# lbcb-sci/raven

Hardware: AMD Instinct MI355X
Metric: read Gbase/s through overlap+polish (higher is better)
Workload: dtype u32

## Files before the change

raven_amd/csrc/poa4.hip:

```cpp
#include <algorithm>
#include <cstddef>
#include <cstdio>
#include <cstdlib>
#include <cstring>
#include <vector>

#include "poa.h"
#include "poa2_window.h"

namespace rvn {

namespace {

struct P4 {
  static constexpr int G = 4, GS = 16, kBand = 32;
  static constexpr int kRing = 22;
  static constexpr int kRowB = 64;
  static constexpr int kMaxD = 8;
  static constexpr int kEdges = 8;
  static constexpr int kEdgesMax = 15;
  static constexpr int kU = 8;
};
constexpr u32 kNone4 = 0xFFFFu;
constexpr i32 kNegU = -0x30000000;
// ... 187 lines not shown
#if defined(__HIP_DEVICE_COMPILE__)
  asm volatile("" : "+v"(p));
#endif
  return p;
}

__host__ __device__ inline u32 group_min_u(u32 v) {
#pragma unroll
  for (int off = 8; off > 0; off >>= 1) {
    const u32 o = static_cast<u32>(sv::bperm(static_cast<int>(v), sv::lane() ^ off));
    v = o < v ? o : v;
  }
  return v;
}
__host__ __device__ inline i32 group_max_i(i32 v) {
#pragma unroll
  for (int off = 8; off > 0; off >>= 1) {
    const i32 o = sv::bperm(v, sv::lane() ^ off);
    v = o > v ? o : v;
  }
  return v;
}

__host__ __device__ inline u32 poa4_nth_pred_rank(const Poa4Slot& sl, u32 v, u32 k, bool full) {
  const Poa2Slot& g = sl.g;
  const u32 c = g.in_cnt[v];
  u32 seen = 0;
  for (u32 i = 0; i < c; ++i) {
    const u32 t = g.in_tail[v * kPoaMaxIn + i];
    if (full || g.mark[t]) {
      if (seen == k) return sl.rb[t] & 0xFFFFu;
      ++seen;
    }
  }
  return 0;
}

__host__ __device__ __forceinline__ u32 mulhi_u32(u32 a, u32 b) {
#if defined(__HIP_DEVICE_COMPILE__)
  return __umulhi(a, b);
#else
  return static_cast<u32>((static_cast<unsigned long long>(a) * b) >> 32);
#endif
}
__host__ __device__ __forceinline__ u32 magic_of(u32 d) { return d <= 1 ? 0u : static_cast<u32>(0x100000000ULL / d) + 1u; }
__host__ __device__ __forceinline__ u32 div_magic(u32 n, u32 m) { return m ? mulhi_u32(n, m) : n; }

struct alignas(16) Poa4LdsDesc {
  u32 segtab[32];
  u32 seq2[60];
  u8 bytes[1024];
};

__host__ __device__ inline void poa4_guide_to_lds(Poa4LdsDesc& S, const PoaLayer* Lp, u32 len, i32 span) {
  const int lane = sv::lane();
  if (lane < 8) {
    const i32 sg = lane;
    const i32 x0 = (sg * span) / 8, x1 = ((sg + 1) * span) / 8;
    const i32 wa = sg == 0 ? 0 : static_cast<i32>(Lp->way[sg - 1]);
    const i32 wb = sg == 7 ? static_cast<i32>(len) : static_cast<i32>(Lp->way[sg]);
    S.segtab[4 * sg] = static_cast<u32>(x0);
    S.segtab[4 * sg + 1] = static_cast<u32>(wa);
    S.segtab[4 * sg + 2] = static_cast<u32>(wb - wa);
    S.segtab[4 * sg + 3] = magic_of(static_cast<u32>(x1 > x0 ? x1 - x0 : 1));
  }
}
template <class K>
__host__ __device__ __forceinline__ i32 poa4_band_start(const Poa4LdsDesc& S, i32 bpos, i32 lb, i32 span, u32 span_magic, u32 len) {
  i32 x = bpos - lb;
  x = x < 0 ? 0 : (x > span ? span : x);
  const u32 seg = div_magic(static_cast<u32>(x) * 8u, span_magic);
  const u32 sg = seg > 7u ? 7u : seg;
  const uint4 st = *reinterpret_cast<const uint4*>(&S.segtab[4 * sg]);
  const i32 dw = static_cast<i32>(st.z);
  const u32 num = static_cast<u32>(x - static_cast<i32>(st.x)) * static_cast<u32>(dw < 0 ? -dw : dw);
  const i32 qn = static_cast<i32>(div_magic(num, st.w));
  i32 b = static_cast<i32>(st.y) + (dw < 0 ? -qn : qn) - K::kBand / 2;
  const i32 bmax = static_cast<i32>(len) + 1 - K::kBand;
  b = b > bmax ? bmax : b;
  b = b < 0 ? 0 : b;
  return (b == bmax && bmax > 0) ? (b + 1) & ~1 : b & ~1;
}

struct Poa4ScoresAny {
  i32 m, n, g;
  __host__ __device__ explicit Poa4ScoresAny(const Poa4Args& A) : m(A.m), n(A.n_), g(A.gp) {}
};
struct Poa4ScoresRacon {
  static constexpr i32 m = 3, n = -5, g = -4;
  __host__ __device__ explicit Poa4ScoresRacon(const Poa4Args&) {}
};
template <class K, class SC>
__host__ __device__ inline void poa4_dp(const Poa4Args A, Poa4Lds& S, unsigned char* slot_mem, bool act, u32 t_end, u32 len,
                                        u32& best_rho1) {
  P4_ASSUME_GLOBAL(slot_mem);
  P4_ASSUME_LDS(&S);
  const int lane = sv::lane();
  const int gl = lane & 15, q = lane >> 4;
  const Poa4Slot sl = poa4_carve(slot_mem, A.nmax, A.lmax);
  {
    const u32 neg = pack16(kNegInf16, kNegInf16);
    for (int idx = gl; idx < K::kRing * kRowW4; idx += 16) lds_st32(S, poa4_ring_byte(q, static_cast<u32>(idx)), neg);
    if (lane < 40) S.neg[lane] = neg;
#if !defined(__HIP_DEVICE_COMPILE__) && defined(RVN_DEBUG_KNOBS)
    if (const char* f = knob("RVN_POA4_RING_FILL")) {
      const int mode = std::atoi(f);
      for (int idx = gl; idx < K::kRing * kRowW4; idx += 16) {
        u32 h = (static_cast<u32>(idx) * 2654435761u) ^ (static_cast<u32>(q) * 40503u) ^ (len * 97u);
        h ^= h >> 13;
        const i32 base = mode == 3 ? 10 : -100, span = mode == 3 ? 50 : 800;
        const i32 lo = mode == 2 ? 28000 : base - static_cast<i32>(h % span), hi = mode == 2 ? 28000 : base - static_cast<i32>((h >> 12) % span);
        if (mode >= 1 && mode <= 3) lds_st32(S, poa4_ring_byte(q, static_cast<u32>(idx)), pack16(lo, hi));
      }
// ... 503 lines not shown
    g.visits[i] = blen >= 2 ? 1 : 0;
    g.order[i] = static_cast<u16>(i);
    rb[i] = i | (i << 16);
    const i32 wgt = poa_layer_weight(A.src, bb, i);
    if (i > 0) {
      const i32 wp = poa_layer_weight(A.src, bb, i - 1);
      g.in_cnt[i] = 1;
      g.in_tail[i * kPoaMaxIn] = static_cast<u16>(i - 1);
      g.in_w[i * kPoaMaxIn] = wp + wgt;
    } else {
      g.in_cnt[i] = 0;
    }
    g.out_cnt[i] = i + 1 < blen ? 1 : 0;
  }
  for (u32 i = blen + lane; i < A.nmax; i += 64) {
    g.in_cnt[i] = 0;
    g.out_cnt[i] = 0;
    g.visits[i] = 0;
  }
  sv::sync();
  return 1;
}

template <class GT>
__host__ __device__ __forceinline__ u32 poa4_letter(const GT& Sg, u32 p) {
  return (Sg.seq2[(p + 1) >> 4] >> (2 * ((p + 1) & 15u))) & 3u;
}

__host__ __device__ __forceinline__ Poa2Slot poa4_graph(unsigned char* slot_mem, u32 nmax, u32 lmax, bool flip) {
  Poa2Slot g = poa4_carve(slot_mem, nmax, lmax).g;
  if (flip) {
    u16* t = g.order;
    g.order = g.order2;
    g.order2 = t;
  }
  return g;
}
__host__ __device__ __forceinline__ void atomic_add_i32(i32* p, i32 v) {
#if defined(__HIP_DEVICE_COMPILE__)
  __hip_atomic_fetch_add(p, v, __ATOMIC_RELAXED, __HIP_MEMORY_SCOPE_WORKGROUP);
#else
  *p += v;
#endif
}
__host__ __device__ __forceinline__ void atomic_inc_u16(u16* base, u32 idx) {
#if defined(__HIP_DEVICE_COMPILE__)
  __hip_atomic_fetch_add(reinterpret_cast<u32*>(base) + (idx >> 1), (idx & 1u) ? 0x10000u : 1u, __ATOMIC_RELAXED,
                         __HIP_MEMORY_SCOPE_WORKGROUP);
#else
  base[idx] += 1;
#endif
}

template <int GW, int UP>
__host__ __device__ inline u32 poa4_update_graph(const Poa4Args A, u16* nslot, const u32* seq2, unsigned char* slot_mem, bool act,
                                                 const PoaLayer* Lp, u32 len, u32 lb, u32& nn, bool& flip,
                                                 unsigned long long& t_add, unsigned long long& t_ord) {
  P4_ASSUME_GLOBAL(slot_mem);
  P4_ASSUME_GLOBAL(Lp);
  P4_ASSUME_LDS(nslot);
  P4_ASSUME_LDS(seq2);
  const int lane = sv::lane();
  const int gl = lane & (GW - 1), gbase = lane & ~(GW - 1);
  constexpr unsigned long long kGMask = GW == 64 ? ~0ULL : ((1ULL << (GW & 63)) - 1ULL);
  auto shift1 = [&](int v, int fill) -> int {
    if constexpr (GW == 16) {
      return sv::row_shr<1>(v, fill);
    } else {
      const int t = sv::bperm(v, lane - 1);
      return gl == 0 ? fill : t;
    }
  };
  auto gmax = [&](i32 v) -> i32 {
    if constexpr (GW == 16) return group_max_i(v);
    else return sv::wave_max(v);
  };
  const Poa2Slot g = poa4_graph(slot_mem, A.nmax, A.lmax, flip);
  const u32* const rb32 = poa4_carve(slot_mem, A.nmax, A.lmax).rb;
  u16* const rb16 = reinterpret_cast<u16*>(poa4_carve(slot_mem, A.nmax, A.lmax).rb);
  const PoaLayer L = *Lp;
  const u32 nmax = A.nmax, lmax = A.lmax;
  unsigned long long t0 = sv::clock();
  const u32 n_old = nn;
  const u32 max_len = static_cast<u32>(sv::wave_max(act ? static_cast<int>(len) : 0));
  auto gballot = [&](bool p) -> unsigned long long { return (sv::ballot(p) >> gbase) & kGMask; };
  auto letter_at = [&](u32 p) -> u32 { return (seq2[(p + 1) >> 4] >> (2 * ((p + 1) & 15u))) & 3u; };
  u32 first_p = 0xFFFFFFFFu;
  for (u32 p0 = 0; p0 < max_len; p0 += UP * GW) {
    if (!sv::any(act && first_p == 0xFFFFFFFFu && p0 < len)) break;
    u32 pn[UP];
#pragma unroll
    for (int u = 0; u < UP; ++u) {
      const u32 p = p0 + static_cast<u32>(GW) * static_cast<u32>(u) + static_cast<u32>(gl);
      pn[u] = (act && p < len) ? g.pos_node[p] : kNone4;
    }
#pragma unroll
    for (int u = 0; u < UP; ++u) {
      const unsigned long long bal = gballot(pn[u] != kNone4);
      if (first_p == 0xFFFFFFFFu && bal) first_p = p0 + static_cast<u32>(GW) * static_cast<u32>(u) + static_cast<u32>(__builtin_ctzll(bal));
    }
  }
  u32 carry_slot = n_old, carry_b = lb;
  if (act && first_p != 0xFFFFFFFFu) {
    const u32 an = g.pos_node[first_p];
    const u32 rb_an = rb32[an];
    u32 r = rb_an & 0xFFFFu;
    const u32 ac = g.al_cnt[an];
    const uint2 al2 = *reinterpret_cast<const uint2*>(g.al + static_cast<size_t>(an) * 4);
    const u32 a0 = al2.x & 0xFFFFu, a1 = al2.x >> 16, a2 = al2.y & 0xFFFFu;
    const u32 r0 = rb32[ac > 0 ? a0 : an] & 0xFFFFu, r1 = rb32[ac > 1 ? a1 : an] & 0xFFFFu, r2 = rb32[ac > 2 ? a2 : an] & 0xFFFFu;
    r = r0 < r ? r0 : r;
    r = r1 < r ? r1 : r;
    r = r2 < r ? r2 : r;
    carry_slot = r;
    carry_b = rb_an >> 16;
  }
  u32 total_new = 0;
  u32 why = 0;
  u32 prev_tgt = kNone4;
  i32 prev_w = 0;
  for (u32 p0 = 0; p0 < max_len; p0 += UP * GW) {
    const bool go = act && why == 0;
    u32 p[UP], an[UP], letter[UP];
    bool valid[UP], has[UP];
#pragma unroll
    for (int u = 0; u < UP; ++u) {
      p[u] = p0 + static_cast<u32>(GW) * static_cast<u32>(u) + static_cast<u32>(gl);
      valid[u] = go && p[u] < len;
      an[u] = valid[u] ? g.pos_node[p[u]] : kNone4;
      letter[u] = valid[u] ? letter_at(p[u]) : 0u;
    }
    u32 c_an[UP], ac[UP], rk_an[UP], bp_an[UP];
    uint2 al2[UP];
    i32 wgt[UP];
#pragma unroll
    for (int u = 0; u < UP; ++u) {
      has[u] = valid[u] && an[u] != kNone4;
      const u32 a = has[u] ? an[u] : 0u;
      c_an[u] = g.code[a];
      ac[u] = g.al_cnt[a];
      const u32 rba = rb32[a];
      rk_an[u] = rba & 0xFFFFu;
      bp_an[u] = rba >> 16;
      al2[u] = *reinterpret_cast<const uint2*>(g.al + static_cast<size_t>(a) * 4);
      wgt[u] = valid[u] ? static_cast<i32>(static_cast<u8>(poa_layer_weight(A.src, L, p[u]))) : 0;
    }
    u32 kt[UP][3], c_kt[UP][3], rk_kt[UP][3];
#pragma unroll
    for (int u = 0; u < UP; ++u) {
      if (!has[u]) ac[u] = 0;
      kt[u][0] = al2[u].x & 0xFFFFu;
      kt[u][1] = al2[u].x >> 16;
      kt[u][2] = al2[u].y & 0xFFFFu;
#pragma unroll
      for (int k = 0; k < 3; ++k) {
        const u32 t = static_cast<u32>(k) < ac[u] ? kt[u][k] : 0u;
        c_kt[u][k] = g.code[t];
        rk_kt[u][k] = rb32[t] & 0xFFFFu;
      }
    }
    u32 tgt[UP], id_new[UP];
    bool is_new[UP];
#pragma unroll
    for (int u = 0; u < UP; ++u) {
      u32 t = kNone4, rmax = rk_an[u];
      if (has[u]) {
        if (c_an[u] == letter[u]) t = an[u];
#pragma unroll
        for (int k = 0; k < 3; ++k) {
          if (static_cast<u32>(k) < ac[u]) {
            rmax = rk_kt[u][k] > rmax ? rk_kt[u][k] : rmax;
            if (t == kNone4 && c_kt[u][k] == letter[u]) t = kt[u][k];
          }
        }
      }
      const u32 gslot = rmax + 1, gb = bp_an[u];
      const unsigned long long bal = gballot(has[u]);
      const unsigned long long below = bal & (gl == 63 ? ~0ULL : ((2ULL << gl) - 1ULL));
      const int src = below ? 63 - __builtin_clzll(below) : 0;
      const u32 s_sh = static_cast<u32>(sv::bperm(static_cast<int>(gslot), gbase | src));
      const u32 b_sh = static_cast<u32>(sv::bperm(static_cast<int>(gb), gbase | src));
      const u32 fslot = below ? s_sh : carry_slot;
      const u32 fb = below ? b_sh : carry_b;
      {
        const int top = bal ? 63 - __builtin_clzll(bal) : 0;
        const u32 cs = static_cast<u32>(sv::bperm(static_cast<int>(gslot), gbase | top));
        const u32 cb = static_cast<u32>(sv::bperm(static_cast<int>(gb), gbase | top));
        if (bal) {
          carry_slot = cs;
          carry_b = cb;
        }
      }
      is_new[u] = valid[u] && t == kNone4;
      const unsigned long long nb = gballot(is_new[u]);
      const u32 cnt = static_cast<u32>(__builtin_popcountll(nb));
      if (go && why == 0 && (n_old + total_new + cnt > nmax || total_new + cnt > lmax)) why = 2;
      id_new[u] = 0;
      if (is_new[u] && why == 0) {
        const u32 tn = total_new + static_cast<u32>(__builtin_popcountll(nb & ((1ULL << gl) - 1ULL)));
        const u32 id = n_old + tn;
        id_new[u] = id;
        t = id;
        nslot[tn] = static_cast<u16>(fslot);
        g.code[id] = static_cast<u8>(letter[u]);
        rb16[2 * static_cast<size_t>(id) + 1] = static_cast<u16>(fb);
        u32 c2 = 0;
        uint2 mine = uint2{0, 0};
        if (has[u]) {
#pragma unroll
          for (int k = 0; k < 3; ++k) {
            if (static_cast<u32>(k) < ac[u]) {
// ... 278 lines not shown
          max_sc = sc;
        }
      }
      if (static_cast<u32>(lane) < rows) lpred[m_it] = static_cast<u16>(predv);
    }
    general = sv::any(bad != 0) || (maxn >= 0 && g.out_cnt[maxn] != 0);
  }
  if (general) {
    sv::sync();
    poa4_consensus_general(g, n_nodes, nmax, win, trim, S, out, out_len);
    return;
  }
  lds_order();
  u32 cl = 0;
  i32 begin = 0, end = -1;
  if (lane == 0) {
    u32 cur = maxn < 0 ? 0xFFFFu : static_cast<u32>(maxn);
    while (cur != 0xFFFFu && cl < kCapNodes) {
      lstack[cl++] = static_cast<u16>(cur);
      cur = lpred[cur];
    }
    end = static_cast<i32>(cl) - 1;
    if (trim) {
      const u32 avg = (win.n_layers - 1) / 2;
      auto cov = [&](i32 pos) -> u32 {
        const u32 v = lstack[cl - 1 - static_cast<u32>(pos)];
        u32 c = g.visits[v];
        for (u32 k = 0; k < g.al_cnt[v]; ++k) c += g.visits[g.al[v * 4 + k]];
        return c;
      };
      for (; begin < static_cast<i32>(cl); ++begin)
        if (cov(begin) >= avg) break;
      for (; end >= 0; --end)
        if (cov(end) >= avg) break;
      if (begin >= end) {
        begin = 0;
        end = static_cast<i32>(cl) - 1;
      }
    }
  }
  cl = static_cast<u32>(sv::rfl(static_cast<int>(cl)));
  begin = sv::rfl(begin);
  end = sv::rfl(end);
  lds_order();
  i32 n_out = end - begin + 1;
  if (n_out < 0) n_out = 0;
  if (static_cast<u32>(n_out) > win.out_cap) n_out = static_cast<i32>(win.out_cap);
  for (i32 p = lane; p < n_out; p += 64) out[p] = g.code[lstack[cl - 1 - static_cast<u32>(begin + p)]];
  if (lane == 0) *out_len = static_cast<u32>(n_out);
}

enum : u32 { kIdle = 0, kRunning = 1, kLayersDone = 2, kFinal = 3, kFailed = 4, kHandedOn = 5 };

struct Poa4Win {
  u32 wi;
  u32 phase, status, nn, n_eff, li, flip;
  u32 act, full, len, lb, span;
  u32 r_lo, n_rows, t_end, best_rho1;
  u32 b_first;
  u32 dflag;
  u32 cells_full, cells_band;
};
static_assert(sizeof(Poa4Win) == 80, "state record");
__host__ __device__ __forceinline__ void atomic_max_u32(u32* p, u32 v) {
#if defined(__HIP_DEVICE_COMPILE__)
  atomicMax(p, v);
#else
  if (v > *p) *p = v;
#endif
}
__host__ __device__ __forceinline__ void atomic_add_u32(u32* p, u32 v) {
#if defined(__HIP_DEVICE_COMPILE__)
  atomicAdd(p, v);
#else
  *p += v;
#endif
}

struct Poa4Ctx {
  Poa4Win* st;
  u32 first;
  u32 count;
  u32 quad_delta;
  u32 gw;
};
__host__ __device__ __forceinline__ u32 poa4_group_windows(const Poa4Ctx& C) { return C.gw ? C.gw : static_cast<u32>(P4::G); }

__host__ __device__ __forceinline__ unsigned char* poa4_slot_of(const Poa4Args& A, const Poa4Ctx&, u32 wave, int q) {
  return A.scratch + (static_cast<size_t>(wave) * P4::G + static_cast<size_t>(q)) * A.slot_bytes;
}
__host__ __device__ __forceinline__ u32 poa4_my_record(const Poa4Ctx& C, u32 wave, int q) {
  const u32 gw = poa4_group_windows(C);
  const u32 pos = (wave + C.quad_delta) * gw + static_cast<u32>(q);
  return (static_cast<u32>(q) < gw && pos < C.count) ? wave * P4::G + static_cast<u32>(q) : 0xFFFFFFFFu;
}
__host__ __device__ __forceinline__ u32 poa4_position(const Poa4Ctx& C, u32 wave, int q) {
  return C.first + (wave + C.quad_delta) * poa4_group_windows(C) + static_cast<u32>(q);
}

__host__ __device__ inline void poa4_phase_init(const Poa4Args& A, const Poa4Ctx& C, u32 wave) {
  const int lane = sv::lane();
  const unsigned long long t_init0 = sv::clock();
  for (int q2 = 0; q2 < P4::G; ++q2) {
    const u32 rec = poa4_my_record(C, wave, q2);
    if (rec == 0xFFFFFFFFu) continue;
    const u32 pos = poa4_position(C, wave, q2);
    const u32 wi = A.sched ? A.sched[pos] : pos;
    const PoaWindow wq = A.windows[wi];
    const Poa4Slot sl2 = poa4_carve(poa4_slot_of(A, C, wave, q2), A.nmax, A.lmax);
    Poa2Slot g = sl2.g;
    u32 nn2 = 0, ne2 = 0;
    const u32 r = poa4_init_window(A, wq, g, sl2.rb, wi, nn2, ne2);
    if (lane == 0) {
      Poa4Win w{};
      w.wi = wi;
      w.phase = r == 1 ? kRunning : kFinal;
      w.status = r == 1 ? 0u : r;
      w.nn = nn2;
      w.n_eff = ne2;
      w.li = 1;
      C.st[rec] = w;
    }
  }
  if (A.phase_cycles && lane == 0) sv::atomic_add(&A.phase_cycles[15], sv::clock() - t_init0);
}

__host__ __device__ inline void poa4_subgraph_marks(Poa2Slot& g, const u32* rb, const u16* order, u32* pend, u32 n_nodes,
                                                    u32 begin, u32 end, u32& r_lo_out, u32& r_hi_out) {
  const int lane = sv::lane();
  for (u32 i = lane; i < n_nodes; i += 64) {
    g.mark[i] = 0;
    g.sub_out[i] = 0;
  }
  for (u32 i = lane; i < 256; i += 64) pend[i] = 0;
  lds_order();
  const u32 end_rank = rb[end] & 0xFFFFu;
  const u32 top_rank = end_rank + 3 < n_nodes ? end_rank + 3 : n_nodes - 1;
  unsigned long long w_cur = 0, w_above = 0, w_low = 0;
  u32 r_lo = 0xFFFFFFFFu, r_hi = 0;
  const i32 top_blk = static_cast<i32>(top_rank >> 6);
  if ((end_rank >> 6) == static_cast<u32>(top_blk)) w_cur = 1ULL << (end_rank & 63u);
  else w_low = 1ULL << (end_rank & 63u);
  for (i32 blk = top_blk; blk >= 0; --blk) {
    const u32 r0 = static_cast<u32>(blk) << 6;
    const u32 r = r0 + static_cast<u32>(lane);
    const bool in = r < n_nodes && r <= top_rank;
    const u32 v = in ? order[r] : 0u;
    u32 c = in ? g.in_cnt[v] : 0u;
    const u32 ac = in ? g.al_cnt[v] : 0u;
    const uint4 ta = *reinterpret_cast<const uint4*>(g.in_tail + static_cast<size_t>(v) * kPoaMaxIn);
    const uint2 al2 = *reinterpret_cast<const uint2*>(g.al + static_cast<size_t>(v) * 4);
    const bool ok = in && v >= begin;
    u32 rec_a = 0, rec_b = 0, rec_f = ok ? 1u : 0u;
#pragma unroll
    for (int k = 0; k < 8; ++k) {
      const u32 wd = k < 2 ? ta.x : (k < 4 ? ta.y : (k < 6 ? ta.z : ta.w));
      const u32 t = static_cast<u32>(k) < c ? (wd >> (16 * (k & 1))) & 0xFFFFu : 0u;
      const u32 rt = rb[t] & 0xFFFFu;
      u32 lb = (static_cast<u32>(k) < c && t >= begin) ? r - rt : 0u;
      if (lb > 254u) {
        lb = 0;
        rec_f |= 2u;
      }
      if (k < 4) rec_a |= lb << (8 * k);
      else rec_b |= lb << (8 * (k - 4));
    }
    if (c > 8) rec_f |= 2u;
#pragma unroll
    for (int k = 0; k < 3; ++k) {
      const u32 m = k == 0 ? al2.x & 0xFFFFu : (k == 1 ? al2.x >> 16 : al2.y & 0xFFFFu);
      const bool has = static_cast<u32>(k) < ac;
      const u32 rm = rb[has ? m : 0u] & 0xFFFFu;
      const i32 d = has ? static_cast<i32>(rm) - static_cast<i32>(r) : 0;
// ... 30 lines not shown
          const u32 lb = ((k < 4 ? a : b) >> (8 * (k & 3))) & 0xFFu;
          if (lb) {
            const int pos = l - static_cast<int>(lb);
            if (pos >= 0) w_cur |= 1ULL << pos;
            else if (pos >= -64) w_low |= 1ULL << (pos + 64);
            else if (lane == 0) pend[(r0 + l - lb) >> 5] |= 1u << ((r0 + l - lb) & 31u);
          }
        }
        if (f & 2u) {
          const u32 vs = order[r0 + static_cast<u32>(l)];
          const u32 cs = g.in_cnt[vs];
          for (u32 k = 0; k < cs; ++k) {
            const u32 t = g.in_tail[vs * kPoaMaxIn + k];
            if (t < begin) continue;
            const u32 rt = rb[t] & 0xFFFFu;
            if (rt >= r0) w_cur |= 1ULL << (rt - r0);
            else if (rt + 64 >= r0) w_low |= 1ULL << (rt + 64 - r0);
            else if (lane == 0) pend[rt >> 5] |= 1u << (rt & 31u);
          }
        }
        lds_order();
      } else {
        w_cur &= ~(1ULL << l);
      }
    }
    if (in && ((w_cur >> lane) & 1ULL)) {
      g.mark[v] = 1;
      r_lo = r < r_lo ? r : r_lo;
      r_hi = r + 1 > r_hi ? r + 1 : r_hi;
    }
    w_above = w_cur;
    w_cur = w_low;
    w_low = 0;
  }
  sv::sync();
  for (u32 v = lane; v < n_nodes; v += 64) {
    if (!g.mark[v]) continue;
    const u32 c = g.in_cnt[v];
    for (u32 k = 0; k < c; ++k) {
      const u32 t = g.in_tail[v * kPoaMaxIn + k];
      if (g.mark[t]) sv::atomic_add(reinterpret_cast<unsigned int*>(g.sub_out) + (t >> 1), (t & 1) ? 0x10000u : 1u);
    }
  }
  {
    const i32 lo_neg = sv::wave_max(r_lo == 0xFFFFFFFFu ? -0x7FFFFFFF : -static_cast<i32>(r_lo));
    const i32 hi = sv::wave_max(static_cast<i32>(r_hi));
    r_lo_out = lo_neg == -0x7FFFFFFF ? 0u : static_cast<u32>(-lo_neg);
    r_hi_out = lo_neg == -0x7FFFFFFF ? 0u : static_cast<u32>(hi);
  }
  sv::sync();
}

template <class K>
__host__ __device__ inline void poa4_phase_setup(const Poa4Args& A, const Poa4Ctx& C, Poa4LdsDesc& S, u32 rec) {
  const int lane = sv::lane();
  const u32 wave_dp = rec / P4::G;
  const int q = static_cast<int>(rec % P4::G);
  if (poa4_my_record(C, wave_dp, q) == 0xFFFFFFFFu) return;
  Poa4Win me = C.st[rec];
  sv::sync();
  if (me.phase != kRunning) return;
  const unsigned long long t0 = sv::clock();
  const PoaWindow wq = A.windows[me.wi];
  u32 liq = me.li;
  while (liq < wq.n_layers &&
         (A.layers[wq.layer_first + liq].len == 0 || (A.src.layer_ok && !A.src.layer_ok[wq.layer_first + liq])))
    ++liq;
  me.act = 0;
  me.li = liq;
  if (liq >= wq.n_layers) {
    me.phase = kLayersDone;
    if (lane == 0) C.st[rec] = me;
    return;
  }
  const PoaLayer L = A.layers[wq.layer_first + liq];
  if (L.len > A.lmax || L.len > static_cast<u32>(kPoa2MaxSeq)) {
    me.phase = kFailed;
    me.status = 4;
    if (lane == 0) C.st[rec] = me;
    return;
  }
  const Poa4Slot sl = poa4_carve(poa4_slot_of(A, C, wave_dp, q), A.nmax, A.lmax);
  Poa2Slot g = sl.g;
  for (u32 i = lane; i < L.len; i += 64) {
    S.bytes[i] = static_cast<u8>(poa_layer_code(A.src, L, i));
    g.pos_node[i] = static_cast<u16>(kNone4);
  }
  lds_order();
  if (lane < 60) {
    u32 x = 0;
    for (u32 c = 0; c < 16; ++c) {
      const i32 p = static_cast<i32>(static_cast<u32>(lane) * 16 + c) - 1;
      if (p >= 0 && p < static_cast<i32>(L.len)) x |= static_cast<u32>(S.bytes[p] & 3u) << (2 * c);
    }
    sl.seq2g[lane] = x;
  }
  const u32 blen = A.layers[wq.layer_first].len;
  const u32 offset = static_cast<u32>(0.01 * blen);
  const bool full = L.begin < offset && L.end > blen - offset;
  u32 r_lo = 0, r_hi = me.nn;
  if (!full) {
    lds_order();
    poa4_subgraph_marks(g, sl.rb, me.flip ? g.order2 : g.order, reinterpret_cast<u32*>(S.bytes), me.nn, L.begin, L.end, r_lo, r_hi);
  }
  const i32 lb = static_cast<i32>(L.begin), span = static_cast<i32>(L.end) - static_cast<i32>(L.begin) + 1;
  poa4_guide_to_lds(S, A.layers + wq.layer_first + liq, L.len, span);
  lds_order();
  if (lane < 32) sl.seq2g[64 + lane] = S.segtab[lane];
  u32 b_first = 0;
  if (r_hi > r_lo) {
    const u32 v0 = (me.flip ? g.order2 : g.order)[r_lo];
    b_first = static_cast<u32>(poa4_band_start<K>(S, static_cast<i32>(sl.rb[v0] >> 16), lb, span,
                                                   magic_of(static_cast<u32>(span > 0 ? span : 1)), L.len));
  }
  me.act = 1;
  me.full = full ? 1u : 0u;
  me.len = L.len;
  me.lb = L.begin;
  me.span = static_cast<u32>(span);
  me.r_lo = r_lo;
  me.n_rows = r_hi - r_lo;
  me.t_end = 0;
  me.best_rho1 = 0;
  me.b_first = b_first;
  me.dflag = 0;
  if (lane == 0) C.st[rec] = me;
  if (A.phase_cycles && lane == 0) sv::atomic_add(&A.phase_cycles[0], sv::clock() - t0);
}

constexpr int kDescPer = 4;
template <class K>
__host__ __device__ inline void poa4_phase_desc_onewave(const Poa4Args& A, const Poa4Ctx& C, Poa4LdsDesc& S, u32 rec) {
  const int lane = sv::lane();
  const u32 wave_dp = rec / P4::G;
  const int q = static_cast<int>(rec % P4::G);
  if (poa4_my_record(C, wave_dp, q) == 0xFFFFFFFFu) return;
  const Poa4Slot sl = poa4_carve(poa4_slot_of(A, C, wave_dp, q), A.nmax, A.lmax);
  const Poa2Slot& g = sl.g;
  const Poa4Win me = C.st[rec];
  if (me.phase != kRunning || !me.act) return;
  const unsigned long long t_desc0 = sv::clock();
  const u32 nn = me.nn;
  const bool full = me.full != 0;
  const u32 len = me.len, r_lo = me.r_lo, n_rows = me.n_rows, r_hi = r_lo + n_rows;
  const i32 lb = static_cast<i32>(me.lb), span = static_cast<i32>(me.span), b_first = static_cast<i32>(me.b_first);
  const u32 span_magic = magic_of(static_cast<u32>(span > 0 ? span : 1));
  const u32 dump_off = poa4_dump_byte(q);
  const u32 neg_off = poa4_neg_byte(q);
  const u32 neg2 = neg_off | (neg_off << 16);
  u32 flag = 0, marked_rows = 0;
  i32 t_end = 0;
  {
    const u32 gw = sl.seq2g[lane < 60 ? lane : 64 + (lane - 60)];
    const u32 gw2 = lane < 28 ? sl.seq2g[68 + lane] : 0u;
    if (lane < 60) S.seq2[lane] = gw;
    else S.segtab[lane - 60] = gw;
    if (lane < 28) S.segtab[4 + lane] = gw2;
  }
  lds_order();
  for (u32 v0 = 0; v0 < nn; v0 += 64 * kDescPer) {
    u32 rbv[kDescPer];
#pragma unroll
    for (int u = 0; u < kDescPer; ++u) {
      const u32 v = v0 + static_cast<u32>(u) * 64 + static_cast<u32>(lane);
      rbv[u] = v < nn ? sl.rb[v] : 0u;
    }
#pragma unroll
    for (int u = 0; u < kDescPer; ++u) {
      const u32 v = v0 + static_cast<u32>(u) * 64 + static_cast<u32>(lane);
      if (v < nn) {
        const i32 b = poa4_band_start<K>(S, static_cast<i32>(rbv[u] >> 16), lb, span, span_magic, len);
        sl.rbl[v] = (rbv[u] & 0xFFFFu) | (static_cast<u32>(b) << 16);
      }
    }
  }
  sv::sync();
  for (u32 v0 = 0; v0 < nn; v0 += 64 * kDescPer) {
    u32 vv[kDescPer], rbv[kDescPer], cc[kDescPer], code[kDescPer], outc_f[kDescPer], outc_s[kDescPer], mk[kDescPer];
    uint4 tl[kDescPer];
#pragma unroll
    for (int u = 0; u < kDescPer; ++u) {
      vv[u] = v0 + static_cast<u32>(u) * 64 + static_cast<u32>(lane);
      const u32 vq = vv[u] < nn ? vv[u] : 0u;
      rbv[u] = sl.rbl[vq];
      cc[u] = g.in_cnt[vq];
      code[u] = g.code[vq];
      outc_f[u] = g.out_cnt[vq];
      outc_s[u] = full ? 0u : g.sub_out[vq];
      mk[u] = full ? 1u : g.mark[vq];
      tl[u] = *reinterpret_cast<const uint4*>(g.in_tail + static_cast<size_t>(vq) * kPoaMaxIn);
    }
    bool ok[kDescPer], marked[kDescPer];
    u32 cmax = 0;
#pragma unroll
    for (int u = 0; u < kDescPer; ++u) {
      const u32 r = rbv[u] & 0xFFFFu;
      ok[u] = vv[u] < nn && r >= r_lo && r < r_hi;
      marked[u] = ok[u] && mk[u] != 0;
      if (!marked[u]) cc[u] = 0;
      cmax = cc[u] > cmax ? cc[u] : cmax;
    }
    cmax = static_cast<u32>(sv::wave_max(static_cast<i32>(cmax)));
    u32 trb[kDescPer][8], tmk[kDescPer][8];
#pragma unroll
    for (int k = 0; k < 8; ++k) {
      if (static_cast<u32>(k) < cmax) {
#pragma unroll
        for (int u = 0; u < kDescPer; ++u) {
          const u32 wd = k < 2 ? tl[u].x : (k < 4 ? tl[u].y : (k < 6 ? tl[u].z : tl[u].w));
          const u32 t = static_cast<u32>(k) < cc[u] ? (wd >> (16 * (k & 1))) & 0xFFFFu : 0u;
          trb[u][k] = sl.rbl[t];
          tmk[u][k] = full ? 1u : g.mark[t];
// ... 49 lines not shown
        const u32 t = g.in_tail[static_cast<size_t>(v) * kPoaMaxIn + k];
        edge(sl.rbl[t], full || g.mark[t] != 0);
      }
      if (np > static_cast<u32>(K::kEdgesMax)) flag = 3;
      if (ok[u]) {
        u32 mm = 0;
        {
          const u32 wi = static_cast<u32>(b) >> 4, sh = 2u * (static_cast<u32>(b) & 15u);
          const u32 x0 = S.seq2[wi], x1 = S.seq2[wi + 1], x2 = S.seq2[wi + 2];
          const u32 pat = code[u] * 0x55555555u;
          const u32 elo = funnel_shr(x1, x0, sh) ^ pat, ehi = funnel_shr(x2, x1, sh) ^ pat;
          auto even_bits = [](u32 y) -> u32 {
            y = ~(y | (y >> 1)) & 0x55555555u;
            y = (y | (y >> 1)) & 0x33333333u;
            y = (y | (y >> 2)) & 0x0F0F0F0Fu;
            y = (y | (y >> 4)) & 0x00FF00FFu;
            y = (y | (y >> 8)) & 0x0000FFFFu;
            return y;
          };
          mm = even_bits(elo) | (even_bits(ehi) << 16);
        }
        i32 sdiff = b - b_first;
        if (sdiff < 0) {
          flag = 7;
          sdiff = 0;
        }
        const u32 Srow = rho + (rho >> 4) + (static_cast<u32>(sdiff) >> 1) + 1u;
        const u32 own = marked[u] ? poa4_ring_byte(q, (rho % static_cast<u32>(K::kRing)) * static_cast<u32>(kRowW4)) : dump_off;
        const bool endn = marked[u] && (full ? outc_f[u] : outc_s[u]) == 0;
        uint4 da, db;
        da.x = (2u * Srow) | (own << 16);
        da.y = v | (static_cast<u32>(b) << 16) | ((np > 15u ? 15u : np) << 26) | (marked[u] ? 1u << 30 : 0u) | (endn ? 1u << 31 : 0u);
        da.z = lbw;
        da.w = ep[0];
        db.x = ep[1];
        db.y = ep[2];
        db.z = ep[3];
        db.w = mm;
        sl.desc[2 * static_cast<size_t>(rho)] = da;
        sl.desc[2 * static_cast<size_t>(rho) + 1] = db;
        t_end = static_cast<i32>(Srow) + 17 > t_end ? static_cast<i32>(Srow) + 17 : t_end;
        if (marked[u]) ++marked_rows;
      }
    }
  }
  if (lane < 32) {
    const size_t rho = static_cast<size_t>(n_rows) + static_cast<size_t>(lane);
    sl.desc[2 * rho] = uint4{kInactiveS | (dump_off << 16), 0u, 0u, neg2};
    sl.desc[2 * rho + 1] = uint4{neg2, neg2, neg2, 0u};
  }
  t_end = sv::wave_max(t_end);
  flag = static_cast<u32>(sv::wave_max(static_cast<i32>(flag)));
  marked_rows = sv::wave_sum(marked_rows);
  if (lane == 0) {
    Poa4Win& w = C.st[rec];
    w.t_end = static_cast<u32>(t_end);
    w.dflag = flag;
    w.cells_full += marked_rows * len;
    w.cells_band += marked_rows * (len + 1 < 32u ? len + 1 : 32u);
  }
  if (A.phase_cycles && lane == 0) sv::atomic_add(&A.phase_cycles[10], sv::clock() - t_desc0);
}

template <class K, class SC>
__host__ __device__ inline void poa4_phase_dp(const Poa4Args& A, const Poa4Ctx& C, Poa4Lds& S, u32 wave) {
  const int lane = sv::lane();
  const int q = lane / K::GS;
  const unsigned long long t0 = sv::clock();
  const u32 my_rec = poa4_my_record(C, wave, q);
  u32 act = 0, t_end = 0, len = 0, li = 0;
  if (my_rec != 0xFFFFFFFFu) {
    Poa4Win& w = C.st[my_rec];
    act = (w.phase == kRunning && w.act) ? 1u : 0u;
    t_end = w.t_end;
    len = w.len;
    li = w.li;
    if (act && (w.dflag || t_end + 8u > poa4_steps(A.nmax, A.lmax))) {
      if ((lane & (K::GS - 1)) == 0) {
        w.phase = kFailed;
        w.status = kPoaBandHit | (li << 8) | ((w.dflag ? (w.dflag & 7u) : 1u) << 24);
        w.act = 0;
      }
      act = 0;
    }
  }
  if (!sv::any(act != 0)) return;
  u32 best_rho1 = 0;
  poa4_dp<K, SC>(A, S, poa4_slot_of(A, C, wave, q), act != 0, t_end, len, best_rho1);
  if (act && (lane & (K::GS - 1)) == 0) {
    Poa4Win& w = C.st[my_rec];
    w.best_rho1 = best_rho1;
    if (best_rho1 == 0) {
      w.phase = kFailed;
      w.status = kPoaBandHit | (li << 8) | (9u << 24);
      w.act = 0;
    }
  }
  if (A.phase_cycles && lane == 0) sv::atomic_add(&A.phase_cycles[1], sv::clock() - t0);
}

template <class K>
__host__ __device__ inline void poa4_phase_tb(const Poa4Args& A, const Poa4Ctx& C, Poa4LdsTb& S, u32 wave) {
  const int lane = sv::lane();
  const int q = lane / K::GS;
  const unsigned long long t0 = sv::clock();
  const u32 my_rec = poa4_my_record(C, wave, q);
  u32 act = 0, r_lo = 0, n_rows = 0, full = 0, len = 0, best = 0, li = 0;
  if (my_rec != 0xFFFFFFFFu) {
    const Poa4Win& w = C.st[my_rec];
    act = (w.phase == kRunning && w.act) ? 1u : 0u;
    r_lo = w.r_lo;
    n_rows = w.n_rows;
    full = w.full;
    len = w.len;
    best = w.best_rho1;
    li = w.li;
  }
  if (!sv::any(act != 0)) return;
  u32 bad = 0, band_hit = 0;
  poa4_traceback<K>(A, S, poa4_slot_of(A, C, wave, q), act != 0, r_lo, n_rows, full != 0, len, best, bad, band_hit);
  if (act && (bad || band_hit) && (lane & (K::GS - 1)) == 0) {
    Poa4Win& w = C.st[my_rec];
    w.phase = kFailed;
    w.status = (bad ? bad : kPoaBandHit) | (li << 8) | ((bad ? 11u : 10u) << 24);
    w.act = 0;
  }
  if (A.phase_cycles && lane == 0) sv::atomic_add(&A.phase_cycles[2], sv::clock() - t0);
}

constexpr int kUpdPer = 2;
struct alignas(16) Poa4LdsUpd {
  u16 nslot[kPoa2MaxSeq + 16];
  u32 seq2[64];
};
template <int UP>
__host__ __device__ inline void poa4_phase_update(const Poa4Args& A, const Poa4Ctx& C, Poa4LdsUpd& S, u32 rec) {
  const int lane = sv::lane();
  const u32 wave_dp = rec / P4::G;
  const int q = static_cast<int>(rec % P4::G);
  if (poa4_my_record(C, wave_dp, q) == 0xFFFFFFFFu) return;
  Poa4Win me = C.st[rec];
  if (me.phase != kRunning) return;
  const bool act = me.act != 0;
  unsigned char* const my_slot = poa4_slot_of(A, C, wave_dp, q);
  if (act && lane < 60) S.seq2[lane] = poa4_carve(my_slot, A.nmax, A.lmax).seq2g[lane];
  lds_order();
  unsigned long long t_add = 0, t_ord = 0;
  u32 nn = me.nn;
  bool flip = me.flip != 0;
  const PoaLayer* Lp = A.layers;
  if (act) Lp = A.layers + A.windows[me.wi].layer_first + me.li;
  const u32 why = poa4_update_graph<64, UP>(A, S.nslot, S.seq2, my_slot, act, Lp, me.len, me.lb, nn, flip, t_add, t_ord);
  if (lane == 0) {
    if (act && why) {
      me.phase = kFailed;
      me.status = why;
    } else if (act) {
      me.nn = nn;
      me.flip = flip ? 1u : 0u;
    }
    me.li = me.li + 1;
    me.act = 0;
    C.st[rec] = me;
  }
  if (A.phase_cycles && lane == 0) {
    sv::atomic_add(&A.phase_cycles[3], t_add);
    sv::atomic_add(&A.phase_cycles[4], t_ord);
  }
}

__host__ __device__ inline void poa4_phase_final(const Poa4Args& A, const Poa4Ctx& C, Poa4Lds& S, u32 wave) {
  const int lane = sv::lane();
  const unsigned long long t0 = sv::clock();
  for (int q2 = 0; q2 < P4::G; ++q2) {
    const u32 rec = poa4_my_record(C, wave, q2);
    if (rec == 0xFFFFFFFFu) continue;
    const Poa4Win w = C.st[rec];
    if (w.phase == kHandedOn) continue;
    PoaWindow wq = A.windows[w.wi];
    u32 st = w.status;
    if (w.phase == kFailed || w.phase == kRunning) {
      poa4_copy_backbone(A, wq, A.layers[wq.layer_first], A.out + wq.out_off, A.out_len + w.wi);
      if (w.phase == kRunning) st = 5;
    } else if (w.phase == kLayersDone) {
      Poa2Slot g = poa4_graph(poa4_slot_of(A, C, wave, q2), A.nmax, A.lmax, w.flip != 0);
      wq.n_layers = w.n_eff;
      poa4_consensus(g, poa4_carve(poa4_slot_of(A, C, wave, q2), A.nmax, A.lmax).rb, w.nn, A.nmax, wq, A.trim, S, A.out + wq.out_off,
                     A.out_len + w.wi);
      sv::sync();
      st = 1;
    }
    if (lane == 0) {
      A.status[w.wi] = st;
      if (A.phase_cycles) {
        sv::atomic_add(&A.phase_cycles[6], static_cast<unsigned long long>(w.cells_full));
        sv::atomic_add(&A.phase_cycles[7], static_cast<unsigned long long>(w.cells_band));
      }
    }
  }
  if (A.phase_cycles && lane == 0) sv::atomic_add(&A.phase_cycles[5], sv::clock() - t0);
}

struct alignas(16) Poa4LdsGraph {
  union {
    Poa4LdsUpd upd;
    Poa4LdsDesc desc;
  } u;
};
template <class K, int UP>
__host__ __device__ inline void poa4_phase_graph(const Poa4Args& A, const Poa4Ctx& C, Poa4LdsGraph& S, u32 rec) {
  const u32 wave_dp = rec / P4::G;
  const int q = static_cast<int>(rec % P4::G);
  if (poa4_my_record(C, wave_dp, q) == 0xFFFFFFFFu) return;
  {
    const Poa4Win me = C.st[rec];
    sv::sync();
    if (me.phase != kRunning) return;
    if (me.act) {
      poa4_phase_update<UP>(A, C, S.u.upd, rec);
      sv::phase_fence();
    }
  }
  poa4_phase_setup<K>(A, C, S.u.desc, rec);
  sv::phase_fence();
  poa4_phase_desc_onewave<K>(A, C, S.u.desc, rec);
}
struct alignas(16) Poa4LdsNw {
  union {
    Poa4Lds dp;
    Poa4LdsTb tb;
  } u;
};
template <class K, class SC>
__host__ __device__ inline void poa4_phase_nw(const Poa4Args& A, const Poa4Ctx& C, Poa4LdsNw& S, u32 wave) {
  poa4_phase_dp<K, SC>(A, C, S.u.dp, wave);
  sv::phase_fence();
  poa4_phase_tb<K>(A, C, S.u.tb, wave);
}

struct alignas(16) Poa4LdsAll {
  union {
    Poa4LdsGraph g;
    Poa4LdsNw n;
    Poa4Lds f;
    p2::Poa2Lds<1> w64;
    p2::Poa2Lds<2> w128;
  } u;
};
static_assert(sizeof(Poa4LdsAll) <= 10240, "sixteen waves per CU");

constexpr u32 kEscEmpty = 0xFFFFFFFFu;
__host__ __device__ __forceinline__ u32 poa4_esc_load(const u32* p) {
#if defined(__HIP_DEVICE_COMPILE__)
  return __hip_atomic_load(p, __ATOMIC_RELAXED, __HIP_MEMORY_SCOPE_AGENT);
#else
  return *p;
#endif
}
__host__ __device__ inline bool poa4_esc_push(const Poa4Args& A, u32 wi) {
#if defined(__HIP_DEVICE_COMPILE__)
  u32 k = __hip_atomic_fetch_add(A.esc, sv::lane() == 0 ? 1u : 0u, __ATOMIC_RELAXED, __HIP_MEMORY_SCOPE_AGENT);
  k = static_cast<u32>(sv::rfl(static_cast<int>(k)));
  if (k >= A.esc_cap) return false;
  if (sv::lane() == 0) __hip_atomic_store(A.esc + 4 + k, wi, __ATOMIC_RELAXED, __HIP_MEMORY_SCOPE_AGENT);
  return true;
#else
  (void)A;
  (void)wi;
  return false;
#endif
}
__host__ __device__ inline u32 poa4_esc_pop(const Poa4Args& A) {
#if defined(__HIP_DEVICE_COMPILE__)
  for (;;) {
    u32 p = static_cast<u32>(sv::rfl(static_cast<int>(poa4_esc_load(A.esc))));
    p = p < A.esc_cap ? p : A.esc_cap;
    const u32 t = static_cast<u32>(sv::rfl(static_cast<int>(poa4_esc_load(A.esc + 1))));
    if (t >= p) return kEscEmpty;
// ... 264 lines not shown
```

Before: 1.435.

## Stage pos_node in LDS and software-pipeline graph-update gathers

Copies the window's pos_node array into LDS with 16-byte vector loads once, and reads it from there in the first-position scan and the main update loop instead of re-reading global memory. Loads for the next block's node code, alignment count, rank and alignment list are prefetched one iteration ahead. When the first aligned position falls in block zero, the carry slot is derived from values already loaded rather than through a separate serial gather chain. This adds LDS footprint and register pressure from the prefetch arrays, and restricts the update path to full-wave groups.

```diff
diff --git a/raven_amd/csrc/poa4.hip b/raven_amd/csrc/poa4.hip
--- a/raven_amd/csrc/poa4.hip
+++ b/raven_amd/csrc/poa4.hip
@@ -879,14 +879,26 @@
 #endif
 }
 
+struct alignas(16) Poa4LdsUpd {
+  u16 nslot[kPoa2MaxSeq + 16];
+  u32 seq2[64];
+  u16 pn[kPoa2MaxSeq + 8];
+};
+static_assert(offsetof(Poa4LdsUpd, pn) % 16 == 0, "16-byte LDS stores");
+
 template <int GW, int UP>
-__host__ __device__ inline u32 poa4_update_graph(const Poa4Args A, u16* nslot, const u32* seq2, unsigned char* slot_mem, bool act,
+__host__ __device__ inline u32 poa4_update_graph(const Poa4Args A, Poa4LdsUpd& S, unsigned char* slot_mem, bool act,
                                                  const PoaLayer* Lp, u32 len, u32 lb, u32& nn, bool& flip,
                                                  unsigned long long& t_add, unsigned long long& t_ord) {
+  static_assert(GW == 64, "the staged pos_node[] below belongs to one window per wave");
+  u16* const nslot = S.nslot;
+  const u32* const seq2 = S.seq2;
+  u16* const pn = S.pn;
   P4_ASSUME_GLOBAL(slot_mem);
   P4_ASSUME_GLOBAL(Lp);
   P4_ASSUME_LDS(nslot);
   P4_ASSUME_LDS(seq2);
+  P4_ASSUME_LDS(pn);
   const int lane = sv::lane();
   const int gl = lane & (GW - 1), gbase = lane & ~(GW - 1);
   constexpr unsigned long long kGMask = GW == 64 ? ~0ULL : ((1ULL << (GW & 63)) - 1ULL);
@@ -912,24 +924,35 @@
   const u32 max_len = static_cast<u32>(sv::wave_max(act ? static_cast<int>(len) : 0));
   auto gballot = [&](bool p) -> unsigned long long { return (sv::ballot(p) >> gbase) & kGMask; };
   auto letter_at = [&](u32 p) -> u32 { return (seq2[(p + 1) >> 4] >> (2 * ((p + 1) & 15u))) & 3u; };
+  {
+    uint4 st[2];
+#pragma unroll
+    for (int k = 0; k < 2; ++k) {
+      const u32 i = static_cast<u32>(lane) + 64u * static_cast<u32>(k);
+      st[k] = (act && 8 * i < len) ? *reinterpret_cast<const uint4*>(g.pos_node + 8 * static_cast<size_t>(i)) : uint4{0, 0, 0, 0};
+    }
+#pragma unroll
+    for (int k = 0; k < 2; ++k) {
+      const u32 i = static_cast<u32>(lane) + 64u * static_cast<u32>(k);
+      if (act && 8 * i < len) *reinterpret_cast<uint4*>(pn + 8 * i) = st[k];
+    }
+  }
+  lds_order();
   u32 first_p = 0xFFFFFFFFu;
   for (u32 p0 = 0; p0 < max_len; p0 += UP * GW) {
     if (!sv::any(act && first_p == 0xFFFFFFFFu && p0 < len)) break;
-    u32 pn[UP];
 #pragma unroll
     for (int u = 0; u < UP; ++u) {
       const u32 p = p0 + static_cast<u32>(GW) * static_cast<u32>(u) + static_cast<u32>(gl);
-      pn[u] = (act && p < len) ? g.pos_node[p] : kNone4;
-    }
-#pragma unroll
-    for (int u = 0; u < UP; ++u) {
-      const unsigned long long bal = gballot(pn[u] != kNone4);
+      const u32 pnu = (act && p < len) ? pn[p] : kNone4;
+      const unsigned long long bal = gballot(pnu != kNone4);
       if (first_p == 0xFFFFFFFFu && bal) first_p = p0 + static_cast<u32>(GW) * static_cast<u32>(u) + static_cast<u32>(__builtin_ctzll(bal));
     }
   }
+  const bool first_in_block0 = first_p < static_cast<u32>(UP * GW);
   u32 carry_slot = n_old, carry_b = lb;
-  if (act && first_p != 0xFFFFFFFFu) {
-    const u32 an = g.pos_node[first_p];
+  if (act && first_p != 0xFFFFFFFFu && !first_in_block0) {
+    const u32 an = pn[first_p];
     const u32 rb_an = rb32[an];
     u32 r = rb_an & 0xFFFFu;
     const u32 ac = g.al_cnt[an];
@@ -946,30 +969,43 @@
   u32 why = 0;
   u32 prev_tgt = kNone4;
   i32 prev_w = 0;
+  u32 an_nx[UP], c_nx[UP], ac_nx[UP], rb_nx[UP];
+  uint2 al_nx[UP];
+  auto level12 = [&](u32 p0) {
+#pragma unroll
+    for (int u = 0; u < UP; ++u) {
+      const u32 pp = p0 + static_cast<u32>(GW) * static_cast<u32>(u) + static_cast<u32>(gl);
+      an_nx[u] = (act && pp < len) ? pn[pp] : kNone4;
+    }
+#pragma unroll
+    for (int u = 0; u < UP; ++u) {
+      const u32 a = an_nx[u] != kNone4 ? an_nx[u] : 0u;
+      c_nx[u] = g.code[a];
+      ac_nx[u] = g.al_cnt[a];
+      rb_nx[u] = rb32[a];
+      al_nx[u] = *reinterpret_cast<const uint2*>(g.al + static_cast<size_t>(a) * 4);
+    }
+  };
+  level12(0);
   for (u32 p0 = 0; p0 < max_len; p0 += UP * GW) {
     const bool go = act && why == 0;
     u32 p[UP], an[UP], letter[UP];
     bool valid[UP], has[UP];
+    u32 c_an[UP], ac[UP], rk_an[UP], bp_an[UP];
+    uint2 al2[UP];
+    i32 wgt[UP];
 #pragma unroll
     for (int u = 0; u < UP; ++u) {
       p[u] = p0 + static_cast<u32>(GW) * static_cast<u32>(u) + static_cast<u32>(gl);
       valid[u] = go && p[u] < len;
-      an[u] = valid[u] ? g.pos_node[p[u]] : kNone4;
+      an[u] = valid[u] ? an_nx[u] : kNone4;
       letter[u] = valid[u] ? letter_at(p[u]) : 0u;
-    }
-    u32 c_an[UP], ac[UP], rk_an[UP], bp_an[UP];
-    uint2 al2[UP];
-    i32 wgt[UP];
-#pragma unroll
-    for (int u = 0; u < UP; ++u) {
       has[u] = valid[u] && an[u] != kNone4;
-      const u32 a = has[u] ? an[u] : 0u;
-      c_an[u] = g.code[a];
-      ac[u] = g.al_cnt[a];
-      const u32 rba = rb32[a];
-      rk_an[u] = rba & 0xFFFFu;
-      bp_an[u] = rba >> 16;
-      al2[u] = *reinterpret_cast<const uint2*>(g.al + static_cast<size_t>(a) * 4);
+      c_an[u] = c_nx[u];
+      ac[u] = ac_nx[u];
+      rk_an[u] = rb_nx[u] & 0xFFFFu;
+      bp_an[u] = rb_nx[u] >> 16;
+      al2[u] = al_nx[u];
       wgt[u] = valid[u] ? static_cast<i32>(static_cast<u8>(poa_layer_weight(A.src, L, p[u]))) : 0;
     }
     u32 kt[UP][3], c_kt[UP][3], rk_kt[UP][3];
@@ -984,6 +1020,27 @@
         const u32 t = static_cast<u32>(k) < ac[u] ? kt[u][k] : 0u;
         c_kt[u][k] = g.code[t];
         rk_kt[u][k] = rb32[t] & 0xFFFFu;
+      }
+    }
+    if (p0 + UP * GW < max_len) level12(p0 + UP * GW);
+    if (p0 == 0) {
+      u32 rmin_sel = 0, b_sel = 0;
+#pragma unroll
+      for (int u = 0; u < UP; ++u) {
+        u32 rmin = rk_an[u];
+#pragma unroll
+        for (int k = 0; k < 3; ++k)
+          if (static_cast<u32>(k) < ac[u]) rmin = rk_kt[u][k] < rmin ? rk_kt[u][k] : rmin;
+        if (static_cast<u32>(u) == first_p / static_cast<u32>(GW)) {
+          rmin_sel = rmin;
+          b_sel = bp_an[u];
+        }
+      }
+      const u32 cs = static_cast<u32>(sv::bperm(static_cast<int>(rmin_sel), gbase | static_cast<int>(first_p & (GW - 1))));
+      const u32 cb = static_cast<u32>(sv::bperm(static_cast<int>(b_sel), gbase | static_cast<int>(first_p & (GW - 1))));
+      if (act && first_in_block0) {
+        carry_slot = cs;
+        carry_b = cb;
       }
     }
     u32 tgt[UP], id_new[UP];
@@ -1909,10 +1966,6 @@
 }
 
 constexpr int kUpdPer = 2;
-struct alignas(16) Poa4LdsUpd {
-  u16 nslot[kPoa2MaxSeq + 16];
-  u32 seq2[64];
-};
 template <int UP>
 __host__ __device__ inline void poa4_phase_update(const Poa4Args& A, const Poa4Ctx& C, Poa4LdsUpd& S, u32 rec) {
   const int lane = sv::lane();
@@ -1930,7 +1983,7 @@
   bool flip = me.flip != 0;
   const PoaLayer* Lp = A.layers;
   if (act) Lp = A.layers + A.windows[me.wi].layer_first + me.li;
-  const u32 why = poa4_update_graph<64, UP>(A, S.nslot, S.seq2, my_slot, act, Lp, me.len, me.lb, nn, flip, t_add, t_ord);
+  const u32 why = poa4_update_graph<64, UP>(A, S, my_slot, act, Lp, me.len, me.lb, nn, flip, t_add, t_ord);
   if (lane == 0) {
     if (act && why) {
       me.phase = kFailed;
```

New measurement: 1.414. 1.5% lower.

## Keep window state in registers across graph phases instead of global round-trips

Applied to the files above, without the earlier changes.

The graph phase now loads the per-window state record once, makes it wave-uniform via readfirstlane, and passes it by reference through update, setup and descriptor phases, writing it back once at the end. This removes repeated global loads and stores of the state record and of the window and layer descriptors. The setup phase also writes the packed sequence and segment table directly into LDS, so the descriptor phase no longer reloads them from global memory. A full phase fence is replaced by an lds_order. The backbone length is cached in the enlarged 96-byte record. The cost is higher register pressure from holding the whole record, plus a larger state struct.

```diff
diff --git a/raven_amd/csrc/poa4.hip b/raven_amd/csrc/poa4.hip
--- a/raven_amd/csrc/poa4.hip
+++ b/raven_amd/csrc/poa4.hip
@@ -263,13 +263,17 @@
   u8 bytes[1024];
 };
 
-__host__ __device__ inline void poa4_guide_to_lds(Poa4LdsDesc& S, const PoaLayer* Lp, u32 len, i32 span) {
+__host__ __device__ inline void poa4_guide_to_lds(Poa4LdsDesc& S, const PoaLayer& L, u32 len, i32 span) {
   const int lane = sv::lane();
   if (lane < 8) {
     const i32 sg = lane;
     const i32 x0 = (sg * span) / 8, x1 = ((sg + 1) * span) / 8;
-    const i32 wa = sg == 0 ? 0 : static_cast<i32>(Lp->way[sg - 1]);
-    const i32 wb = sg == 7 ? static_cast<i32>(len) : static_cast<i32>(Lp->way[sg]);
+    i32 wa = 0, wb = static_cast<i32>(len);
+#pragma unroll
+    for (int i = 0; i < 7; ++i) {
+      if (sg == i + 1) wa = static_cast<i32>(L.way[i]);
+      if (sg == i) wb = static_cast<i32>(L.way[i]);
+    }
     S.segtab[4 * sg] = static_cast<u32>(x0);
     S.segtab[4 * sg + 1] = static_cast<u32>(wa);
     S.segtab[4 * sg + 2] = static_cast<u32>(wb - wa);
@@ -1368,7 +1372,7 @@
 
 enum : u32 { kIdle = 0, kRunning = 1, kLayersDone = 2, kFinal = 3, kFailed = 4, kHandedOn = 5 };
 
-struct Poa4Win {
+struct alignas(16) Poa4Win {
   u32 wi;
   u32 phase, status, nn, n_eff, li, flip;
   u32 act, full, len, lb, span;
@@ -1376,8 +1380,17 @@
   u32 b_first;
   u32 dflag;
   u32 cells_full, cells_band;
+  u32 blen;
+  u32 pad_[3];
 };
-static_assert(sizeof(Poa4Win) == 80, "state record");
+static_assert(sizeof(Poa4Win) == 96, "state record");
+__host__ __device__ __forceinline__ void poa4_win_uniform(Poa4Win& w) {
+  auto uni = [](u32& x) { x = static_cast<u32>(sv::rfl(static_cast<int>(x))); };
+  uni(w.wi); uni(w.phase); uni(w.status); uni(w.nn); uni(w.n_eff); uni(w.li); uni(w.flip);
+  uni(w.act); uni(w.full); uni(w.len); uni(w.lb); uni(w.span);
+  uni(w.r_lo); uni(w.n_rows); uni(w.t_end); uni(w.best_rho1);
+  uni(w.b_first); uni(w.dflag); uni(w.cells_full); uni(w.cells_band); uni(w.blen);
+}
 __host__ __device__ __forceinline__ void atomic_max_u32(u32* p, u32 v) {
 #if defined(__HIP_DEVICE_COMPILE__)
   atomicMax(p, v);
@@ -1435,6 +1448,7 @@
       w.nn = nn2;
       w.n_eff = ne2;
       w.li = 1;
+      w.blen = A.layers[wq.layer_first].len;
       C.st[rec] = w;
     }
   }
@@ -1571,35 +1585,29 @@
 }
 
 template <class K>
-__host__ __device__ inline void poa4_phase_setup(const Poa4Args& A, const Poa4Ctx& C, Poa4LdsDesc& S, u32 rec) {
+__host__ __device__ inline void poa4_phase_setup(const Poa4Args& A, Poa4LdsDesc& S, unsigned char* my_slot, Poa4Win& me, const PoaWindow& wq) {
   const int lane = sv::lane();
-  const u32 wave_dp = rec / P4::G;
-  const int q = static_cast<int>(rec % P4::G);
-  if (poa4_my_record(C, wave_dp, q) == 0xFFFFFFFFu) return;
-  Poa4Win me = C.st[rec];
-  sv::sync();
   if (me.phase != kRunning) return;
   const unsigned long long t0 = sv::clock();
-  const PoaWindow wq = A.windows[me.wi];
   u32 liq = me.li;
-  while (liq < wq.n_layers &&
-         (A.layers[wq.layer_first + liq].len == 0 || (A.src.layer_ok && !A.src.layer_ok[wq.layer_first + liq])))
+  PoaLayer L{};
+  while (liq < wq.n_layers) {
+    L = A.layers[wq.layer_first + liq];
+    if (!(L.len == 0 || (A.src.layer_ok && !A.src.layer_ok[wq.layer_first + liq]))) break;
     ++liq;
+  }
   me.act = 0;
   me.li = liq;
   if (liq >= wq.n_layers) {
     me.phase = kLayersDone;
-    if (lane == 0) C.st[rec] = me;
     return;
   }
-  const PoaLayer L = A.layers[wq.layer_first + liq];
   if (L.len > A.lmax || L.len > static_cast<u32>(kPoa2MaxSeq)) {
     me.phase = kFailed;
     me.status = 4;
-    if (lane == 0) C.st[rec] = me;
     return;
   }
-  const Poa4Slot sl = poa4_carve(poa4_slot_of(A, C, wave_dp, q), A.nmax, A.lmax);
+  const Poa4Slot sl = poa4_carve(my_slot, A.nmax, A.lmax);
   Poa2Slot g = sl.g;
   for (u32 i = lane; i < L.len; i += 64) {
     S.bytes[i] = static_cast<u8>(poa_layer_code(A.src, L, i));
@@ -1613,8 +1621,9 @@
       if (p >= 0 && p < static_cast<i32>(L.len)) x |= static_cast<u32>(S.bytes[p] & 3u) << (2 * c);
     }
     sl.seq2g[lane] = x;
-  }
-  const u32 blen = A.layers[wq.layer_first].len;
+    S.seq2[lane] = x;
+  }
+  const u32 blen = me.blen;
   const u32 offset = static_cast<u32>(0.01 * blen);
   const bool full = L.begin < offset && L.end > blen - offset;
   u32 r_lo = 0, r_hi = me.nn;
@@ -1623,7 +1632,7 @@
     poa4_subgraph_marks(g, sl.rb, me.flip ? g.order2 : g.order, reinterpret_cast<u32*>(S.bytes), me.nn, L.begin, L.end, r_lo, r_hi);
   }
   const i32 lb = static_cast<i32>(L.begin), span = static_cast<i32>(L.end) - static_cast<i32>(L.begin) + 1;
-  poa4_guide_to_lds(S, A.layers + wq.layer_first + liq, L.len, span);
+  poa4_guide_to_lds(S, L, L.len, span);
   lds_order();
   if (lane < 32) sl.seq2g[64 + lane] = S.segtab[lane];
   u32 b_first = 0;
@@ -1643,20 +1652,15 @@
   me.best_rho1 = 0;
   me.b_first = b_first;
   me.dflag = 0;
-  if (lane == 0) C.st[rec] = me;
   if (A.phase_cycles && lane == 0) sv::atomic_add(&A.phase_cycles[0], sv::clock() - t0);
 }
 
 constexpr int kDescPer = 4;
 template <class K>
-__host__ __device__ inline void poa4_phase_desc_onewave(const Poa4Args& A, const Poa4Ctx& C, Poa4LdsDesc& S, u32 rec) {
+__host__ __device__ inline void poa4_phase_desc_onewave(const Poa4Args& A, Poa4LdsDesc& S, unsigned char* my_slot, int q, Poa4Win& me) {
   const int lane = sv::lane();
-  const u32 wave_dp = rec / P4::G;
-  const int q = static_cast<int>(rec % P4::G);
-  if (poa4_my_record(C, wave_dp, q) == 0xFFFFFFFFu) return;
-  const Poa4Slot sl = poa4_carve(poa4_slot_of(A, C, wave_dp, q), A.nmax, A.lmax);
+  const Poa4Slot sl = poa4_carve(my_slot, A.nmax, A.lmax);
   const Poa2Slot& g = sl.g;
-  const Poa4Win me = C.st[rec];
   if (me.phase != kRunning || !me.act) return;
   const unsigned long long t_desc0 = sv::clock();
   const u32 nn = me.nn;
@@ -1669,14 +1673,6 @@
   const u32 neg2 = neg_off | (neg_off << 16);
   u32 flag = 0, marked_rows = 0;
   i32 t_end = 0;
-  {
-    const u32 gw = sl.seq2g[lane < 60 ? lane : 64 + (lane - 60)];
-    const u32 gw2 = lane < 28 ? sl.seq2g[68 + lane] : 0u;
-    if (lane < 60) S.seq2[lane] = gw;
-    else S.segtab[lane - 60] = gw;
-    if (lane < 28) S.segtab[4 + lane] = gw2;
-  }
-  lds_order();
   for (u32 v0 = 0; v0 < nn; v0 += 64 * kDescPer) {
     u32 rbv[kDescPer];
 #pragma unroll
@@ -1832,13 +1828,10 @@
   t_end = sv::wave_max(t_end);
   flag = static_cast<u32>(sv::wave_max(static_cast<i32>(flag)));
   marked_rows = sv::wave_sum(marked_rows);
-  if (lane == 0) {
-    Poa4Win& w = C.st[rec];
-    w.t_end = static_cast<u32>(t_end);
-    w.dflag = flag;
-    w.cells_full += marked_rows * len;
-    w.cells_band += marked_rows * (len + 1 < 32u ? len + 1 : 32u);
-  }
+  me.t_end = static_cast<u32>(t_end);
+  me.dflag = flag;
+  me.cells_full += marked_rows * len;
+  me.cells_band += marked_rows * (len + 1 < 32u ? len + 1 : 32u);
   if (A.phase_cycles && lane == 0) sv::atomic_add(&A.phase_cycles[10], sv::clock() - t_desc0);
 }
 
@@ -1914,35 +1907,27 @@
   u32 seq2[64];
 };
 template <int UP>
-__host__ __device__ inline void poa4_phase_update(const Poa4Args& A, const Poa4Ctx& C, Poa4LdsUpd& S, u32 rec) {
+__host__ __device__ inline void poa4_phase_update(const Poa4Args& A, Poa4LdsUpd& S, unsigned char* my_slot, Poa4Win& me, const PoaWindow& wq) {
   const int lane = sv::lane();
-  const u32 wave_dp = rec / P4::G;
-  const int q = static_cast<int>(rec % P4::G);
-  if (poa4_my_record(C, wave_dp, q) == 0xFFFFFFFFu) return;
-  Poa4Win me = C.st[rec];
   if (me.phase != kRunning) return;
   const bool act = me.act != 0;
-  unsigned char* const my_slot = poa4_slot_of(A, C, wave_dp, q);
   if (act && lane < 60) S.seq2[lane] = poa4_carve(my_slot, A.nmax, A.lmax).seq2g[lane];
   lds_order();
   unsigned long long t_add = 0, t_ord = 0;
   u32 nn = me.nn;
   bool flip = me.flip != 0;
   const PoaLayer* Lp = A.layers;
-  if (act) Lp = A.layers + A.windows[me.wi].layer_first + me.li;
+  if (act) Lp = A.layers + wq.layer_first + me.li;
   const u32 why = poa4_update_graph<64, UP>(A, S.nslot, S.seq2, my_slot, act, Lp, me.len, me.lb, nn, flip, t_add, t_ord);
-  if (lane == 0) {
-    if (act && why) {
-      me.phase = kFailed;
-      me.status = why;
-    } else if (act) {
-      me.nn = nn;
-      me.flip = flip ? 1u : 0u;
-    }
-    me.li = me.li + 1;
-    me.act = 0;
-    C.st[rec] = me;
-  }
+  if (act && why) {
+    me.phase = kFailed;
+    me.status = why;
+  } else if (act) {
+    me.nn = nn;
+    me.flip = flip ? 1u : 0u;
+  }
+  me.li = me.li + 1;
+  me.act = 0;
   if (A.phase_cycles && lane == 0) {
     sv::atomic_add(&A.phase_cycles[3], t_add);
     sv::atomic_add(&A.phase_cycles[4], t_ord);
@@ -1992,18 +1977,21 @@
   const u32 wave_dp = rec / P4::G;
   const int q = static_cast<int>(rec % P4::G);
   if (poa4_my_record(C, wave_dp, q) == 0xFFFFFFFFu) return;
-  {
-    const Poa4Win me = C.st[rec];
-    sv::sync();
-    if (me.phase != kRunning) return;
-    if (me.act) {
-      poa4_phase_update<UP>(A, C, S.u.upd, rec);
-      sv::phase_fence();
-    }
-  }
-  poa4_phase_setup<K>(A, C, S.u.desc, rec);
-  sv::phase_fence();
-  poa4_phase_desc_onewave<K>(A, C, S.u.desc, rec);
+  Poa4Win me = C.st[rec];
+  sv::sync();
+  poa4_win_uniform(me);
+  if (me.phase != kRunning) return;
+  const PoaWindow wq = A.windows[me.wi];
+  unsigned char* const my_slot = poa4_slot_of(A, C, wave_dp, q);
+  if (me.act) {
+    poa4_phase_update<UP>(A, S.u.upd, my_slot, me, wq);
+    poa4_win_uniform(me);
+    sv::phase_fence();
+  }
+  poa4_phase_setup<K>(A, S.u.desc, my_slot, me, wq);
+  lds_order();
+  poa4_phase_desc_onewave<K>(A, S.u.desc, my_slot, q, me);
+  if (sv::lane() == 0) C.st[rec] = me;
 }
 struct alignas(16) Poa4LdsNw {
   union {
```

Result: faster. 1.423 before, 1.445 after, median of 6 (+1.6%).
